# paulvantieghem/curla

Hardware: AMD Instinct MI355X
Metric: SAC+CURL gradient updates/sec, batch=512 84x84x9 (higher is better)
Workload: dtype f32

## Files before the change

curla_amd/_lib.py:

```python
import ctypes
import os

_HERE = os.path.dirname(os.path.abspath(__file__))
LIB_PATH = os.environ.get("CURLA_LIB_PATH") or os.path.join(_HERE, "libcurla_hip.so")

c_int, c_ll, c_float, c_size_t, vp = ctypes.c_int, ctypes.c_longlong, ctypes.c_float, ctypes.c_size_t, ctypes.c_void_p
c_u64 = ctypes.c_ulonglong
c_double = ctypes.c_double

ABI_VERSION = 8

SIGNATURES = {
    "curla_conv1_fwd": [vp, c_int, vp, vp, vp, vp, vp, vp, c_int, c_int, c_int, c_int, c_int, c_int, c_int, c_float, vp],
    "curla_conv3x3_s1_fwd": [vp, vp, vp, vp, c_int, c_int, c_int, c_int, vp],
    "curla_conv3x3_s1_fwd2": [vp, vp, vp, vp, c_int, vp, vp, vp, vp, c_int, c_int, c_int, c_int, vp],
    "curla_conv3x3_s1_fwd_stack": [c_int, vp, vp, vp, vp, c_int, vp, vp, vp, vp, c_int, c_int, c_int, c_int, vp],
    "curla_conv3x3_s1_stack_granule": [],
    "curla_conv1_fwd2": [vp, vp, vp, vp, vp, vp, vp, c_int, vp, vp, vp, vp, vp, vp, c_int, c_int, c_int, c_int, c_int, c_int,
                         c_int, c_float, vp],
    "curla_conv3x3_s1_dgrad": [vp, vp, vp, vp, c_int, c_int, c_int, c_int, vp],
    "curla_conv3x3_s1_wgrad": [vp, vp, vp, vp, vp, c_int, c_int, c_int, c_int, vp],
    "curla_conv1_wgrad": [vp, c_int, vp, vp, vp, vp, vp, vp, vp, c_int, c_int, c_int, c_int, c_int, c_int, c_int,
                          c_float, vp],
    "curla_conv3x3_s1_wgrad_slabs": [vp, vp, vp, c_int, c_int, c_int, c_int, vp, vp],
    "curla_conv1_wgrad_slabs": [vp, c_int, vp, vp, vp, vp, vp, c_int, c_int, c_int, c_int, c_int, c_int, c_int, c_float, vp,
                                vp],
    "curla_conv3x3_s1_bwd_slabs": [vp, vp, vp, vp, vp, c_int, c_int, c_int, c_int, vp, vp],
    "curla_conv1_dgrad": [vp, vp, vp, c_int, c_int, c_int, c_int, c_int, c_float, vp],
    "curla_wgrad_reduce_multi": [c_int, vp, vp, vp, vp, vp, vp, vp],
    "curla_conv_wgrad_workspace_floats": [c_int],
    "curla_gemm": [vp, c_int, c_int, c_ll, vp, c_int, c_int, c_ll, vp, c_int, c_ll, c_int, c_int, c_int, c_int, c_int,
                   c_ll, c_float, vp, c_ll, c_int, vp, c_int, c_ll, vp],
    "curla_fc_dx": [vp, vp, vp, vp, c_int, c_int, c_int, vp],
    "curla_fc_dw": [vp, vp, vp, c_int, c_int, c_int, vp],
    "curla_fc_bwd": [vp, vp, vp, vp, vp, c_int, c_int, c_int, vp],
    "curla_fc_bwd_ln": [vp, vp, vp, vp, vp, c_int, c_int, c_int, vp, c_int, vp, vp, vp, vp],
    "curla_fc_dw_ln": [vp, vp, vp, c_int, c_int, c_int, vp, c_int, vp, vp, vp, vp],
    "curla_fc_bwd_ln2": [vp, vp, vp, vp, vp, c_int, c_int, c_int, vp, c_int, vp, vp, vp, vp, c_int, c_int, vp, vp],
    "curla_curl_head": [vp, vp, vp, vp, vp, vp, c_int, c_int, vp, vp, vp, vp, vp, vp, vp, vp, vp, vp],
    "curla_gemm_nested": [vp, c_int, c_int, c_ll, c_ll, vp, c_int, c_int, c_ll, c_ll, vp, c_int, c_ll, c_ll, c_int, c_int, c_int,
                          c_int, c_int, c_float, vp, c_ll, c_ll, c_int, vp, c_int, c_ll, c_ll, vp],
    "curla_mlp_out_fwd_nested": [vp, c_ll, c_ll, vp, c_ll, c_ll, vp, c_ll, c_ll, vp, c_ll, c_ll, c_int, c_int, c_int, c_int, c_int,
                                 vp],
# ... 175 lines not shown
```

curla_amd/csrc/conv.hip:

```cpp
#include <algorithm>
#include <cstdlib>
#include <cstring>
#include <mutex>
#include <type_traits>

#include "common.h"
#include "options.h"

namespace {

constexpr int kLdsPix = 36;

enum { MODE_FWD = 0, MODE_DGRAD = 1 };

__device__ float g_zero_px[32];

#ifdef CURLA_ABLATE
int g_ablate = 0;
#define ABL(bit) (a.dbg & (bit))
#define ABL_HOST g_ablate
#else
#define ABL(bit) 0
#define ABL_HOST 0
#endif
// ... 23 lines not shown
    __syncthreads();
    rw43::run_layer<MODE_FWD, 4>(A.g[l], A.p[l][0], A.p[l][1], lds, blockIdx.x, gridDim.x);
    if (l + 1 < A.nlayers) {
      __builtin_amdgcn_fence(__ATOMIC_RELEASE, "workgroup");
      __syncthreads();
      __builtin_amdgcn_fence(__ATOMIC_ACQUIRE, "workgroup");
    }
  }
}

__global__ __launch_bounds__(256, 1) __attribute__((amdgpu_waves_per_eu(1, 1))) void conv_rw43_dgrad_kernel(rw::Args A) {
  extern __shared__ __attribute__((aligned(16))) float lds[];
  rw43::build_filter<MODE_DGRAD, 256>(lds, A.p[0][0].w, nullptr, threadIdx.x);
  __syncthreads();
  rw43::run_layer<MODE_DGRAD, 4>(A.g[0], A.p[0][0], A.p[0][1], lds, blockIdx.x, gridDim.x);
}

#include "conv_rwb.h"

#ifdef RWB_CLOCK
__device__ unsigned long long g_rwb_clock[3 * 1024];
#endif

template <int NW>
__device__ __forceinline__ void rwb_fwd_body(const rw::Args& A) {
  extern __shared__ __attribute__((aligned(16))) unsigned short lds_h[];
#if defined(RWB_STAMP) || defined(RWB_CLOCK)
  const unsigned long long kt0 = __builtin_readcyclecounter(), kr0 = __builtin_amdgcn_s_memrealtime();
#endif
  for (int l = 0; l < A.nlayers; ++l) {
#ifdef RWB_STAMP
    const unsigned long long k0 = __builtin_readcyclecounter();
#endif
    rwb::build_filter<MODE_FWD, 64 * NW>(lds_h, A.p[l][0].w, A.p[l][1].B > 0 ? A.p[l][1].w : nullptr, threadIdx.x);
    __syncthreads();
#ifdef RWB_STAMP
    const unsigned long long k1 = __builtin_readcyclecounter();
#endif
    rwb::run_layer<MODE_FWD, NW>(A.g[l], A.p[l][0], A.p[l][1], lds_h, blockIdx.x, gridDim.x);
#ifdef RWB_STAMP
    const unsigned long long k2 = __builtin_readcyclecounter();
#endif
    if (l + 1 < A.nlayers) {
      __builtin_amdgcn_fence(__ATOMIC_RELEASE, "workgroup");
      __syncthreads();
      __builtin_amdgcn_fence(__ATOMIC_ACQUIRE, "workgroup");
    }
#ifdef RWB_STAMP
    const unsigned long long k3 = __builtin_readcyclecounter();
    if (threadIdx.x == 0 && blockIdx.x == 7) {
      rwb::g_rwb_stamp[4] += k1 - k0, rwb::g_rwb_stamp[5] += k2 - k1, rwb::g_rwb_stamp[6] += k3 - k2, rwb::g_rwb_stamp[7] += 1;
    }
#endif
  }
#ifdef RWB_STAMP
  if (threadIdx.x == 0 && blockIdx.x == 7) {
    rwb::g_rwb_stamp[15] += __builtin_readcyclecounter() - kt0;
    rwb::g_rwb_stamp[14] += __builtin_amdgcn_s_memrealtime() - kr0;
  }
#endif
#ifdef RWB_CLOCK
  if (threadIdx.x == 0 && blockIdx.x < 1024) {
    g_rwb_clock[3 * blockIdx.x + 0] += __builtin_readcyclecounter() - kt0;
    g_rwb_clock[3 * blockIdx.x + 1] += __builtin_amdgcn_s_memrealtime() - kr0;
    g_rwb_clock[3 * blockIdx.x + 2] += 1;
  }
#endif
}

__global__ __launch_bounds__(512, 1) void conv_rwb_fwd_kernel(rw::Args A) { rwb_fwd_body<8>(A); }

__global__ __launch_bounds__(512, 1) void conv_rwb_dgrad_kernel(rw::Args A) {
  extern __shared__ __attribute__((aligned(16))) unsigned short lds_h[];
  rwb::build_filter<MODE_DGRAD, 512>(lds_h, A.p[0][0].w, nullptr, threadIdx.x);
  __syncthreads();
  rwb::run_layer<MODE_DGRAD, 8>(A.g[0], A.p[0][0], A.p[0][1], lds_h, blockIdx.x, gridDim.x);
}

__global__ __launch_bounds__(256, 2) void conv_rw_dgrad_kernel(rw::Args A) {
  extern __shared__ __attribute__((aligned(16))) float lds[];
  rw::build_filter<MODE_DGRAD, 256>(lds, A.p[0][0].w, nullptr, threadIdx.x);
  __syncthreads();
  rw::run_layer<MODE_DGRAD, 4>(A.g[0], A.p[0][0], A.p[0][1], lds, blockIdx.x, gridDim.x);
}

#include "conv1_rw.h"

template <int C>
__global__ __launch_bounds__(512, 2) void conv1_rw_fwd_kernel(rw::Conv1Args a) {
  rw::conv1_body<C, 8>(a, blockIdx.x, gridDim.x);
}

template <int C>
__global__ __launch_bounds__(512, 2) void wgrad1_rw_kernel(rw::Wgrad1Args a) {
  rw::wgrad1_body<C, 8>(a, blockIdx.x, gridDim.x);
}

// ... 44 lines not shown
    rw::wgrad_body<4>(wa, bid, nblk);
}

__global__ __launch_bounds__(256, 2) void wgrad_rw_kernel(rw::WgradArgs wa) {
  wgrad_any(wa, blockIdx.x, gridDim.x);
}

__global__ __launch_bounds__(256, 2) void bwd_rw2_kernel(rw::WgradArgs wa, rw::Args da, int nw) {
  if ((int)blockIdx.x < nw) {
    wgrad_any(wa, blockIdx.x, nw);
  } else {
    extern __shared__ __attribute__((aligned(16))) float lds[];
    rw::build_filter<MODE_DGRAD, 256>(lds, da.p[0][0].w, nullptr, threadIdx.x);
    __syncthreads();
    rw::run_layer<MODE_DGRAD, 4>(da.g[0], da.p[0][0], da.p[0][1], lds, (int)blockIdx.x - nw, (int)gridDim.x - nw);
  }
}

__global__ __launch_bounds__(256, 2) void bwd_rwb2_kernel(rw::WgradArgs wa, rw::Args da, int nw) {
  if ((int)blockIdx.x < nw) {
    wgrad_any(wa, blockIdx.x, nw);
  } else {
    extern __shared__ __attribute__((aligned(16))) unsigned short lds_hb[];
    rwb::build_filter<MODE_DGRAD, 256>(lds_hb, da.p[0][0].w, nullptr, threadIdx.x);
    __syncthreads();
    rwb::run_layer<MODE_DGRAD, 4>(da.g[0], da.p[0][0], da.p[0][1], lds_hb, (int)blockIdx.x - nw, (int)gridDim.x - nw);
  }
}

#include "conv1_wgrad.h"

#include "conv_wgrad_reduce.h"

constexpr int kMaxLds = 160 * 1024;
static_assert(2 * rwb::kWBytes <= kMaxLds, "the two problems' split filters of conv_rwb_fwd_kernel must fit one CU's LDS");
template <typename K>
int set_lds(K kernel, size_t bytes) {
  if (bytes > (size_t)kMaxLds) return CURLA_ERR_UNSUPPORTED;
  return curla_set_dyn_lds(reinterpret_cast<const void*>(kernel), kMaxLds);
}

template <typename... Params, typename... Args>
int launch(void (*kernel)(Params...), int grid, int threads, size_t lds, hipStream_t st, const Args&... args) {
  if (lds) {
    const int rc = set_lds(kernel, lds);
    if (rc != CURLA_OK) return rc;
  }
// ... 53 lines not shown
  return one_band && Wc * C <= 64 * 16 && opt != kConv1U8Band ? Conv1U8Form::Hybrid : Conv1U8Form::Band;
}

enum class Conv1F32Form { Rw, Band };
Conv1F32Form select_conv1_f32_form(int src_kind, int C, int Hc, int Wc) {
  const bool rw = src_kind == kSrcF32Nhwc && curla_opt(kOptConv1F32) == kConv1F32Rw && (long long)Hc * Wc * C * 4 < (1LL << 30);
  return rw ? Conv1F32Form::Rw : Conv1F32Form::Band;
}

enum class Wgrad1U8Form { B16, F32, F32FourWave };
constexpr size_t kWgrad1U8BandBudget = 76 * 1024, kWgrad1U8BandBudget4 = 38 * 1024;
Wgrad1U8Form select_wgrad1_u8_form(int C, int Wc, int Wo) {
  if ((ABL_HOST & 1024) && (size_t)(2 * 4 + 1) * u8_row_bytes(Wc, C) <= kWgrad1U8BandBudget4) return Wgrad1U8Form::F32FourWave;
  return curla_opt(kOptWgrad1U8) != kWgrad1U8F32 && Wo >= 8 && 3 * C <= 32 ? Wgrad1U8Form::B16 : Wgrad1U8Form::F32;
}

bool rw_supported(int Hi, int Wi) { return (long long)(Hi + 2) * (Wi + 2) * 128 < (1LL << 30); }

rw::Geom s1_plan(S1Form f, int Hi, int Wi, int Ho, int Wo) {
  return f == S1Form::B3 ? rwb::plan(Hi, Wi, Ho, Wo) : f == S1Form::F43 ? rw43::plan(Hi, Wi, Ho, Wo) : rw::plan(Hi, Wi, Ho, Wo);
}
size_t s1_filter_bytes(S1Form f) {
  return f == S1Form::B3 ? rwb::kWBytes : (f == S1Form::F43 ? rw43::kWFloats : rw::kWFloats) * sizeof(float);
}

int launch_rw_fwd(int nlayers, const float* in, const float* const* w, const float* const* bias, float* const* out, int B,
                  const float* in2, const float* const* w2, const float* const* bias2, float* const* out2, int B2, int Hi,
                  int Wi, bool owned, hipStream_t st) {
  const S1Form form = select_s1_form();
  rw::Args A;
  A.nlayers = nlayers;
  for (int l = 0; l < rw::kMaxLayers; ++l) {
    const bool on = l < nlayers;
    const int hi = Hi - 2 * l, wi = Wi - 2 * l;
    A.g[l] = on ? s1_plan(form, hi, wi, hi - 2, wi - 2) : rw::Geom{};
    A.p[l][0] = on ? rw::Problem{l == 0 ? in : out[l - 1], w[l], bias[l], out[l], B} : rw::Problem{};
    A.p[l][1] = (on && B2 > 0) ? rw::Problem{l == 0 ? in2 : out2[l - 1], w2[l], bias2[l], out2[l], B2} : rw::Problem{};
    if (on && (hi < 3 || wi < 3)) return CURLA_ERR_UNSUPPORTED;
  }
  if (!rw_supported(Hi, Wi)) return CURLA_ERR_UNSUPPORTED;
  const int cus = curla_cu_count();
  const int grid = owned ? cus : std::min(B > B2 ? B : B2, cus);
  const size_t lds = (size_t)(B2 > 0 ? 2 : 1) * s1_filter_bytes(form);
  switch (form) {
    case S1Form::B3: return launch(conv_rwb_fwd_kernel, grid, 512, lds, st, A);
    case S1Form::F43: return launch(conv_rw43_fwd_kernel, grid, 256, lds, st, A);
    default: return launch(conv_rw_fwd_kernel, grid, 512, lds, st, A);
  }
}

rw::Args rw_dgrad_args(S1Form form, const float* g, const float* w, const float* act_below, float* gin, int B, int Ho,
                       int Wo) {
  rw::Args A;
  A.nlayers = 1;
  for (int l = 0; l < rw::kMaxLayers; ++l) A.g[l] = rw::Geom{}, A.p[l][0] = rw::Problem{}, A.p[l][1] = rw::Problem{};
  A.g[0] = s1_plan(form, Ho, Wo, Ho + 2, Wo + 2);
  A.p[0][0] = rw::Problem{g, w, act_below, gin, B};
  return A;
}

int launch_dgrad(S1Form form, const float* g, const float* w, const float* act_below, float* gin, int B, int Ho, int Wo,
                 hipStream_t st) {
  const rw::Args A = rw_dgrad_args(form, g, w, act_below, gin, B, Ho, Wo);
  const int cus = curla_cu_count();
  const size_t lds = s1_filter_bytes(form);
  switch (form) {
    case S1Form::B3: return launch(conv_rwb_dgrad_kernel, std::min(B, cus), 512, lds, st, A);
    case S1Form::F43: return launch(conv_rw43_dgrad_kernel, std::min(B, cus), 256, lds, st, A);
    default: return launch(conv_rw_dgrad_kernel, std::min(B, 2 * cus), 256, lds, st, A);
  }
}

int launch_conv_s1(int mode, const float* in, const float* w, const float* aux, float* out, int B, int Hs, int Ws,
                   hipStream_t st, const float* in2 = nullptr, const float* w2 = nullptr, const float* aux2 = nullptr,
                   float* out2 = nullptr, int B2 = 0) {
  if (!rw_supported(Hs, Ws)) return CURLA_ERR_UNSUPPORTED;
  if (mode == MODE_FWD) return launch_rw_fwd(1, in, &w, &aux, &out, B, in2, &w2, &aux2, &out2, B2, Hs, Ws, false, st);
  return launch_dgrad(select_s1_form(), in, w, aux, out, B, Hs, Ws, st);
}

rw::WgradArgs wgrad_args(const float* in, const float* g, float* workspace, int B, int Hi, int Wi, int Ho, int Wo) {
  const bool two_d = select_s1_wgrad_form() == S1WgradForm::XY;
  return rw::WgradArgs{in, g, workspace, B, Hi, Wi, Ho, Wo, two_d ? rw::plan4p(Hi, Wi, Ho, Wo) : rw::plan4(Hi, Wi, Ho, Wo),
                       two_d ? 1 : 0};
}

// ... 149 lines not shown
  return launch_conv_s1(MODE_FWD, in, w, bias, out, B, Hi, Wi, static_cast<hipStream_t>(stream), in2, w2, bias2, out2, B2);
}

int curla_conv3x3_s1_fwd_stack(int nlayers, const float* in, const float* const* w, const float* const* bias,
                               float* const* out, int B, const float* in2, const float* const* w2,
                               const float* const* bias2, float* const* out2, int B2, int Hi, int Wi, int channels,
                               void* stream) {
  CURLA_REQUIRE(nlayers > 0 && nlayers <= rw::kMaxLayers && in && w && bias && out && B > 0 && Hi >= 3 && Wi >= 3);
  CURLA_REQUIRE(B2 == 0 || (in2 && w2 && bias2 && out2));
  if (channels != 32) return CURLA_ERR_UNSUPPORTED;
  const int G1 = curla_cu_count();
  if (B % G1 != 0 || B2 % G1 != 0) return CURLA_ERR_UNSUPPORTED;
  CURLA_REQUIRE(aligned16(in) && (!B2 || aligned16(in2)));
  for (int l = 0; l < nlayers; ++l) {
    CURLA_REQUIRE(w[l] && bias[l] && out[l] && aligned16(w[l]) && aligned16(bias[l]) && aligned16(out[l]));
    CURLA_REQUIRE(!B2 || (w2[l] && bias2[l] && out2[l] && aligned16(w2[l]) && aligned16(bias2[l]) && aligned16(out2[l])));
  }
  if (Hi - 2 * nlayers < 1 || Wi - 2 * nlayers < 1) return CURLA_ERR_UNSUPPORTED;
  return launch_rw_fwd(nlayers, in, w, bias, out, B, in2, w2, bias2, out2, B2, Hi, Wi, true,
                       static_cast<hipStream_t>(stream));
}

int curla_conv3x3_s1_stack_granule(void) { return curla_cu_count(); }

int curla_conv3x3_s1_dgrad(const float* g, const float* w, const float* act_below, float* gin, int B, int Ho, int Wo,
                           int channels, void* stream) {
  CURLA_REQUIRE(g && w && act_below && gin && B > 0 && Ho >= 1 && Wo >= 1);
  if (channels != 32) return gen_dgrad(g, w, act_below, gin, B, Ho, Wo, channels, static_cast<hipStream_t>(stream));
  CURLA_REQUIRE(aligned16(g) && aligned16(gin) && aligned16(act_below) && aligned16(w));
  return launch_conv_s1(MODE_DGRAD, g, w, act_below, gin, B, Ho, Wo, static_cast<hipStream_t>(stream));
}

static int conv1_common_check(const void* src, int src_kind, int B, int C, int Hs, int Ws, int Hc, int Wc) {
  CURLA_REQUIRE(src && B > 0 && Hc >= 3 && Wc >= 3 && src_kind >= 0 && src_kind <= 2);
  if (C != 9 && C != 12 && C != 6 && C != 3) return CURLA_ERR_UNSUPPORTED;
  if (src_kind == kSrcU8Ring) {
    CURLA_REQUIRE(Hs >= Hc && Ws >= Wc);
    CURLA_REQUIRE((reinterpret_cast<uintptr_t>(src) & 3) == 0);
  }
  return CURLA_OK;
}

struct Conv1Second {
  const int64_t* idx;
  const int32_t* h1;
  const int32_t* w1;
// ... 144 lines not shown
  CURLA_REQUIRE(nslabs);
  return launch_wgrad_s1(in, g, workspace, B, Hi, Wi, channels, static_cast<hipStream_t>(stream), nslabs);
}

int curla_conv3x3_s1_bwd_slabs(const float* in, const float* g, const float* w, float* gin, float* workspace, int B, int Hi,
                               int Wi, int channels, int* nslabs, void* stream) {
  CURLA_REQUIRE(in && g && w && gin && workspace && nslabs && B > 0 && Hi >= 3 && Wi >= 3);
  hipStream_t st = static_cast<hipStream_t>(stream);
  if (channels != 32) {
    const int rc = gen_wgrad_s1(in, g, workspace, B, Hi, Wi, channels, st, nslabs);
    return rc != CURLA_OK ? rc : gen_dgrad(g, w, in, gin, B, Hi - 2, Wi - 2, channels, st);
  }
  CURLA_REQUIRE(aligned16(in) && aligned16(g) && aligned16(w) && aligned16(gin));
  const int Ho = Hi - 2, Wo = Wi - 2;
  if (!rw_supported(Hi, Wi)) return CURLA_ERR_UNSUPPORTED;
  const S1Form form = select_s1_form();
  if (form == S1Form::F43) {
    const int rc = launch_wgrad_s1(in, g, workspace, B, Hi, Wi, channels, st, nslabs);
    return rc != CURLA_OK ? rc : launch_dgrad(form, g, w, in, gin, B, Ho, Wo, st);
  }
  const int per_cu = select_bwd_shape(form, B, Ho, Wo) == BwdShape::SideBySide ? 1 : 2;
  const int n = std::min(B, per_cu * curla_cu_count());
  const rw::WgradArgs wr = wgrad_args(in, g, workspace, B, Hi, Wi, Ho, Wo);
  const rw::Args dr = rw_dgrad_args(form, g, w, in, gin, B, Ho, Wo);
  const size_t lds = std::max<size_t>(s1_filter_bytes(form), kPartialS1 * sizeof(float));
  *nslabs = n;
  return launch(form == S1Form::B3 ? bwd_rwb2_kernel : bwd_rw2_kernel, 2 * n, 256, lds, st, wr, dr, n);
}

int curla_wgrad_reduce_multi(int njobs, const float* const* slabs, const int* nslabs, const int* nw, const int* nb,
                             float* const* dw, float* const* db, void* stream) {
  CURLA_REQUIRE(njobs > 0 && njobs <= kMaxReduceJobs && slabs && nslabs && nw && dw && db);
  ReduceJobs J;
  int blocks = 0;
  for (int j = 0; j < njobs; ++j) {
    CURLA_REQUIRE(slabs[j] && dw[j] && db[j] && nslabs[j] > 0 && nw[j] > 0);
    J.partial[j] = slabs[j], J.dw[j] = dw[j], J.db[j] = db[j], J.nslabs[j] = nslabs[j], J.nw[j] = nw[j];
    J.nb[j] = nb ? nb[j] : 32;
    CURLA_REQUIRE(J.nb[j] > 0);
    J.first_block[j] = blocks;
    blocks += (nw[j] + J.nb[j] + 31) / 32;
  }
  J.first_block[njobs] = blocks;
  J.njobs = njobs;
  return launch(wgrad_reduce_multi_kernel, blocks, 1024, 0, static_cast<hipStream_t>(stream), J);
}

// ... 71 lines not shown
```

curla_amd/csrc/conv_rw.h:

```cpp
#pragma once

namespace rw {

constexpr int kWFloats = 3 * 4 * 2 * 2 * 256;

__device__ __forceinline__ __amdgpu_buffer_rsrc_t uniform_rsrc(const void* p, int bytes) {
  const unsigned long long a = reinterpret_cast<unsigned long long>(p);
  const unsigned lo32 = __builtin_amdgcn_readfirstlane((unsigned)a);
  const unsigned hi32 = __builtin_amdgcn_readfirstlane((unsigned)(a >> 32));
  return __builtin_amdgcn_make_buffer_rsrc(reinterpret_cast<void*>(((unsigned long long)hi32 << 32) | lo32), (short)0,
                                           __builtin_amdgcn_readfirstlane(bytes), 0x00020000);
}

struct Geom {
  int Hi, Wi;
  int Ho, Wo;
  int nfull;
  int brem;
  int nr;
  int nseg;
  int ntr;
  int steps;
};

struct Problem {
  const float* in;
  const float* w;
  const float* aux;
  float* out;
  int B;
};

constexpr int kMaxLayers = 6;
struct Args {
  int nlayers;
  Geom g[kMaxLayers];
  Problem p[kMaxLayers][2];
};

inline void plan_units(Geom& g, int Ho, int cols, int per) {
  g.nfull = cols / per, g.brem = cols % per;
  g.nr = g.nseg = g.ntr = 0;
  if (g.brem) {
    long best = -1;
    for (int nr = 1; nr <= Ho; ++nr) {
      const int nseg = (Ho + nr - 1) / nr;
      const int ntr = (g.brem * nseg + per - 1) / per;
      const long cost = (long)ntr * nr * 64 + (long)ntr * 2 * 8;
      if (best < 0 || cost <= best) best = cost, g.nr = nr, g.nseg = nseg, g.ntr = ntr;
    }
  }
  g.steps = g.nfull * Ho + g.ntr * g.nr;
}

inline Geom plan(int Hi, int Wi, int Ho, int Wo) {
  Geom g;
  g.Hi = Hi, g.Wi = Wi, g.Ho = Ho, g.Wo = Wo;
  plan_units(g, Ho, (Wo + 1) / 2, 16);
  return g;
}
// ... 228 lines not shown
```

curla_amd/csrc/conv_rwb.h:

```cpp
#pragma once

namespace rwb {

using rw::Args;
using rw::Geom;
using rw::Problem;
using rw::uniform_rsrc;

typedef short bf16x8 __attribute__((ext_vector_type(8)));
typedef unsigned u32x4 __attribute__((ext_vector_type(4)));
typedef __bf16 bf16x2_t __attribute__((ext_vector_type(2)));

constexpr int kWBytes = 3 * 4 * 2 * 3 * 64 * 16;

inline Geom plan(int Hi, int Wi, int Ho, int Wo) { return rw::plan(Hi, Wi, Ho, Wo); }

struct B3 {
  u32x4 h, m, l;
};

__device__ __forceinline__ unsigned cvt_pk_bf16(float x0, float x1) {
  const f32x2 v = {x0, x1};
  return __builtin_bit_cast(unsigned, __builtin_convertvector(v, bf16x2_t));
}
// ... 2 lines not shown
  B3 o;
#if defined(RWB_ABL) && (RWB_ABL & 1)
#pragma unroll
  for (int p = 0; p < 4; ++p) o.h[p] = __builtin_bit_cast(unsigned, v[2 * p]), o.m[p] = __builtin_bit_cast(unsigned, v[2 * p + 1]);
  o.l = o.h;
  return o;
#endif
#pragma unroll
  for (int p = 0; p < 4; ++p) {
    const float x0 = v[2 * p], x1 = v[2 * p + 1];
    const unsigned h = cvt_pk_bf16(x0, x1);
    const float r0 = x0 - __builtin_bit_cast(float, h << 16), r1 = x1 - __builtin_bit_cast(float, h & 0xFFFF0000u);
    const unsigned m = cvt_pk_bf16(r0, r1);
    const float s0 = r0 - __builtin_bit_cast(float, m << 16), s1 = r1 - __builtin_bit_cast(float, m & 0xFFFF0000u);
    o.h[p] = h, o.m[p] = m, o.l[p] = cvt_pk_bf16(s0, s1);
  }
  return o;
}

__device__ __forceinline__ f32x4 mfma_bf16(const u32x4 a, const u32x4 b, const f32x4 c) {
  return __builtin_amdgcn_mfma_f32_16x16x32_bf16(__builtin_bit_cast(bf16x8, a), __builtin_bit_cast(bf16x8, b), c, 0, 0, 0);
}

template <int MODE, int NT>
__device__ __forceinline__ void build_filter(unsigned short* lds_w, const float* __restrict__ w0,
                                             const float* __restrict__ w1, int tid) {
  const int nitems = (w1 ? 2 : 1) * 6 * 64;
  for (int item = tid; item < nitems; item += NT) {
    const int slot = item & 63, dm = (item >> 6) % 6, prob = item / 384;
    const int li = slot & 15, kq = slot >> 4, dy = dm >> 1, mt = dm & 1;
    const float* __restrict__ w = prob ? w1 : w0;
    const int co = 16 * mt + li;
    float u[8][4];
#pragma unroll
    for (int j = 0; j < 8; ++j) {
      const int ci = 8 * kq + j;
      const float* t = MODE == MODE_FWD ? w + (co * 32 + ci) * 9 + dy * 3 : w + (ci * 32 + co) * 9 + (2 - dy) * 3;
      if (MODE == MODE_FWD)
        rw::filter_transform(t[0], t[1], t[2], u[j]);
      else
        rw::filter_transform(t[2], t[1], t[0], u[j]);
    }
    u32x4* img = reinterpret_cast<u32x4*>(lds_w + prob * (kWBytes / 2));
#pragma unroll
    for (int pos = 0; pos < 4; ++pos) {
      float v[8];
#pragma unroll
      for (int j = 0; j < 8; ++j) v[j] = u[j][pos];
      const B3 x = split8(v);
      u32x4* p = img + ((((dy * 4 + pos) * 2 + mt) * 3)) * 64 + slot;
      p[0] = x.h, p[64] = x.m, p[128] = x.l;
    }
  }
}

#ifdef RWB_STAMP
__device__ unsigned long long g_rwb_stamp[16];
#endif

struct Acc {
  f32x4 m[2][4];
};

template <int MODE, int NW>
__device__ __forceinline__ void run_layer(const Geom& G, const Problem& P0, const Problem& P1, const unsigned short* lds_w,
                                          int bid, int nblk) {
  const int lane = threadIdx.x & 63;
  const int wave = __builtin_amdgcn_readfirstlane(threadIdx.x >> 6);
  const int li = lane & 15, kq = lane >> 4;
  const int pad = MODE == MODE_FWD ? 0 : 2;
  const int cnt0 = bid < P0.B ? (P0.B - bid + nblk - 1) / nblk : 0;
  const int cnt1 = bid < P1.B ? (P1.B - bid + nblk - 1) / nblk : 0;
  const int nstrips = G.nfull + G.ntr;
  const int T = (cnt0 + cnt1) * G.steps;
  const int lo = (int)((long)wave * T / NW), hi = (int)((long)(wave + 1) * T / NW);
  const int in_row = G.Wi * 128, out_row = G.Wo * 128;

// ... 192 lines not shown
```

curla_amd/csrc/options.h:

```cpp
#pragma once

enum CurlaOpt {
  kOptConv1U8 = 0,
  kOptConv1F32,
  kOptS1Fwd,
  kOptBwdSplit,
  kOptGemmTile,
  kOptLinearBwd,
  kOptGemmMfma,
  kOptS1Wgrad,
  kOptWgrad1U8,
  kOptCount
};

enum Conv1U8Opt { kConv1U8Auto, kConv1U8Hybrid, kConv1U8Band, kConv1U8Rw, kConv1U8Rwb, kConv1U8Values };
enum Conv1F32Opt { kConv1F32Rw, kConv1F32Band, kConv1F32Values };
enum S1FwdOpt { kS1FwdAuto, kS1FwdF23, kS1FwdF43, kS1FwdB3, kS1FwdValues };
enum BwdSplitOpt { kBwdSplitAuto, kBwdSplitOff, kBwdSplitOn, kBwdSplitValues };
enum GemmTileOpt { kGemmTileAuto, kGemmTile6464, kGemmTile6432, kGemmTile3232, kGemmTile12864, kGemmTileValues };
enum LinearBwdOpt { kLinearBwdPair, kLinearBwdSplit, kLinearBwdValues };
enum GemmMfmaOpt { kGemmMfmaAuto, kGemmMfmaF32, kGemmMfmaB3, kGemmMfmaValues };
enum S1WgradOpt { kS1WgradAuto, kS1WgradX, kS1WgradXY, kS1WgradValues };
enum Wgrad1U8Opt { kWgrad1U8Auto, kWgrad1U8F32, kWgrad1U8B16, kWgrad1U8Values };

int curla_opt(int id);
```

curla_amd/csrc/options.hip:

```cpp
#include "options.h"

#include <atomic>
#include <cctype>
#include <cstdlib>
#include <cstring>
#include <mutex>

#include "../../include/curla_hip.h"

namespace {

struct OptDef {
  const char* name;
  const char* values[6];
  const char* alias[6];
};

constexpr OptDef kDefs[kOptCount] = {
    {"conv1_u8", {"auto", "hybrid", "band", "rw", "rwb", nullptr}, {nullptr, nullptr, nullptr, nullptr, nullptr, nullptr}},
    {"conv1_f32", {"rw", "band", nullptr}, {nullptr, nullptr, nullptr}},
    {"s1_fwd", {"auto", "f23", "f43", "b3", nullptr}, {nullptr, nullptr, nullptr, "bf16x3", nullptr}},
    {"bwd_split", {"auto", "0", "1", nullptr}, {nullptr, "off", "on", nullptr}},
    {"gemm_tile", {"auto", "6464", "6432", "3232", "12864", nullptr}, {nullptr, "64x64", "64x32", "32x32", "128x64", nullptr}},
    {"linear_bwd", {"pair", "split", nullptr}, {nullptr, nullptr, nullptr}},
    {"gemm_mfma", {"auto", "f32", "b3", nullptr}, {nullptr, nullptr, "bf16x3", nullptr}},
    {"s1_wgrad", {"auto", "x", "xy", nullptr}, {nullptr, "1d", "2d", nullptr}},
    {"wgrad1_u8", {"auto", "f32", "b16", nullptr}, {nullptr, nullptr, "bf16", nullptr}},
};

constexpr int kValueCount[kOptCount] = {kConv1U8Values, kConv1F32Values, kS1FwdValues, kBwdSplitValues, kGemmTileValues,
                                        kLinearBwdValues, kGemmMfmaValues, kS1WgradValues, kWgrad1U8Values};
constexpr bool value_counts_match() {
  for (int id = 0; id < kOptCount; ++id)
    if (!kDefs[id].values[kValueCount[id] - 1] || kDefs[id].values[kValueCount[id]]) return false;
  return true;
}
static_assert(value_counts_match(), "options.h names a different number of values than kDefs lists for some option");

std::atomic<int> g_value[kOptCount];
std::once_flag g_once;

int parse(const OptDef& d, const char* text) {
  for (int i = 0; i < 6 && d.values[i]; ++i)
    if (!strcmp(text, d.values[i]) || (d.alias[i] && !strcmp(text, d.alias[i]))) return i;
  return -1;
}

void init_from_env() {
  for (int id = 0; id < kOptCount; ++id) {
    char env[64] = "CURLA_";
    size_t n = strlen(env);
    for (const char* p = kDefs[id].name; *p && n + 1 < sizeof(env); ++p) env[n++] = (char)toupper((unsigned char)*p);
    env[n] = 0;
    const char* e = getenv(env);
// ... 39 lines not shown
```

curla_amd/curl_sac.py:

```python
import os
import warnings

import numpy as np
import torch
import torch.nn as nn

from . import autograd, ops
from .augmentations import RandomCrop
from .encoder import CNNEncoder
from .ops import ObsRef
from .optim import FlatAdam

LOG_FREQ = 25_000


def weight_init(m):
    if isinstance(m, nn.Linear):
        nn.init.orthogonal_(m.weight.data)
        if m.bias is not None:
            m.bias.data.zero_()
        return
    if isinstance(m, (nn.Conv2d, nn.ConvTranspose2d)):
        kh, kw = m.weight.shape[2:]
        assert kh == kw, "square kernels only"
# ... 699 lines not shown
        B, F, K, L = obs_ref.B, enc.feature_dim, enc.flat_dim, enc.num_layers
        acts = ws.acts_main
        dy, dy2 = (dz, None) if twin_ld is None else (dz[0], dz[1])
        streams = ops.fc_bwd_streams(F, K)
        ln = ln_token if ln_token is not None else ops.ln_bwd(
            dy, xhat, rstd, enc.ln.weight, B, F, ws.dfc, dgamma=enc.ln.weight.grad, dbeta=enc.ln.bias.grad,
            dbias_in=enc.fc.bias.grad, dy2=dy2, ld=twin_ld, defer=ws.ln_partial if streams else None)
        h = acts[-1]
        cur = L % 2
        g = ws.gviews[cur][L - 1]
        if streams and conv_grads:
            ops.fc_bwd(ws.dfc, enc.fc.weight, h, g, enc.fc.weight.grad, B, F, K, ln=ln)
        elif streams:
            ops.fc_dw(ws.dfc, h, enc.fc.weight.grad, B, F, K, ln=ln)
        else:
            ops.linear_dw(ws.dfc, 0, h, 0, enc.fc.weight.grad, 0, B, F, K)
        if dense_done is not None:
            dense_done()
        if not conv_grads:
            return
        if not streams:
            ops.linear_dx(ws.dfc, 0, enc.fc.weight, 0, g, 0, B, F, K, mask=h)
        jobs = []
        for layer in range(L, 1, -1):
            conv = enc.convs[layer - 1]
            cur ^= 1
            gin = ws.gviews[cur][layer - 2]
            n = ops.conv_s1_bwd_slabs(acts[layer - 2], g, conv.weight, gin, ws.wg_ws[layer - 1])
            jobs.append((ws.wg_ws[layer - 1], n, conv.weight.grad, conv.bias.grad))
            g = gin
        n = ops.conv1_wgrad_slabs(obs_ref, g, ws.wg_ws[0], enc.num_filters)
        jobs.append((ws.wg_ws[0], n, enc.convs[0].weight.grad, enc.convs[0].bias.grad))
        for i in range(0, len(jobs), 8):
            ops.wgrad_reduce_multi(jobs[i:i + 8])

    def _records(self, step):
        return self.log_param_hist_imgs and step % LOG_FREQ == 0

    def _noise(self, ws, noise):
        if noise is not None:
            ws.noise.copy_(noise)
            return ws.noise, None
        if self._graph_cap is not None:
            cap = self._graph_cap
            addr = cap["rng"][cap["n_noise"]]
            cap["n_noise"] += 1
# ... 564 lines not shown
```

curla_amd/ops.py:

```python
import ctypes

import torch

from . import _lib
from ._lib import call, ptr, stream

F32 = torch.float32


def _dev(t, dtype=F32):
    if not ((t.is_cuda or _lib._trace_hook is not None) and t.dtype == dtype and t.is_contiguous()):
        raise _lib.CurlaHipError(f"expected a contiguous {dtype} CUDA tensor, got {t.dtype} {t.device} "
                                 f"contiguous={t.is_contiguous()}")
    return t


class ObsRef:

    __slots__ = ("src", "is_u8", "idx", "h1", "w1", "B", "C", "Hs", "Ws", "Hc", "Wc", "guard", "pair")

    def __init__(self):
        self.guard = None
        self.pair = None

# ... 99 lines not shown
def cu_count():
    if _lib._trace_hook is not None:
        return 256
    return _device_cached("cus", lambda: torch.cuda.get_device_properties(torch.cuda.current_device()).multi_processor_count)


def conv1_pairable(o1: "ObsRef", o2: "ObsRef"):
    return (o1.is_u8 == 1 and o2.is_u8 == 1 and o1.src.data_ptr() == o2.src.data_ptr() and o1.src.shape == o2.src.shape
            and (o1.Hc, o1.Wc) == (o2.Hc, o2.Wc))


def conv1_fwd2(o1: "ObsRef", w, b, out, o2: "ObsRef", w2, b2, out2, scale=1.0 / 255.0):
    o1.check(), o2.check()
    call("curla_conv1_fwd2", ptr(o1.src), ptr(o1.idx), ptr(o1.h1), ptr(o1.w1), ptr(w), ptr(b), ptr(out), o1.B, ptr(o2.idx),
         ptr(o2.h1), ptr(o2.w1), ptr(w2), ptr(b2), ptr(out2), o2.B, o1.C, o1.Hs, o1.Ws, o1.Hc, o1.Wc, w.shape[0], scale,
         stream())


def conv_s1_dgrad(g, w, act_below, gin):
    B, H, W, C = g.shape
    call("curla_conv3x3_s1_dgrad", ptr(g), ptr(w), ptr(act_below), ptr(gin), B, H, W, C, stream())


def conv_s1_wgrad(x, g, dw, db, ws):
    B, H, W, C = x.shape
    call("curla_conv3x3_s1_wgrad", ptr(x), ptr(g), ptr(dw), ptr(db), ptr(ws), B, H, W, C, stream())


def conv_s1_wgrad_slabs(x, g, ws):
    import ctypes
    B, H, W, C = x.shape
    n = ctypes.c_int(1)
    call("curla_conv3x3_s1_wgrad_slabs", ptr(x), ptr(g), ptr(ws), B, H, W, C, ctypes.addressof(n), stream())
    return n.value


def conv_s1_bwd_slabs(x, g, w, gin, ws):
    import ctypes
    B, H, W, C = x.shape
    n = ctypes.c_int(1)
    call("curla_conv3x3_s1_bwd_slabs", ptr(x), ptr(g), ptr(w), ptr(gin), ptr(ws), B, H, W, C, ctypes.addressof(n),
         stream())
    return n.value


def conv1_wgrad_slabs(obs: ObsRef, g, ws, channels, scale=1.0 / 255.0):
# ... 486 lines not shown
```

include/curla_hip.h:

```cpp
#ifndef CURLA_HIP_H
#define CURLA_HIP_H

#include <stddef.h>
#include <stdint.h>

#ifdef __cplusplus
extern "C" {
#endif

#define CURLA_OK 0
#define CURLA_ERR_ARG (-1)
#define CURLA_ERR_LAUNCH (-2)
#define CURLA_ERR_UNSUPPORTED (-3)

const char* curla_version(void);

#define CURLA_ABI_VERSION 8
int curla_abi_version(void);

int curla_set_option(const char* name, const char* value);
const char* curla_get_option(const char* name);


int curla_conv1_fwd(const void* src, int src_kind, const int64_t* idx, const int32_t* h1, const int32_t* w1,
// ... 9 lines not shown
int curla_conv3x3_s1_fwd2(const float* in, const float* w, const float* bias, float* out, int B, const float* in2,
                          const float* w2, const float* bias2, float* out2, int B2, int Hi, int Wi, int channels,
                          void* stream);
int curla_conv3x3_s1_fwd_stack(int nlayers, const float* in, const float* const* w, const float* const* bias,
                               float* const* out, int B, const float* in2, const float* const* w2,
                               const float* const* bias2, float* const* out2, int B2, int Hi, int Wi, int channels,
                               void* stream);
int curla_conv3x3_s1_stack_granule(void);

int curla_conv3x3_s1_dgrad(const float* g, const float* w, const float* act_below, float* gin, int B, int Ho, int Wo,
                           int channels, void* stream);
int curla_conv3x3_s1_wgrad(const float* in, const float* g, float* dw, float* db, float* workspace, int B, int Hi,
                           int Wi, int channels, void* stream);
int curla_conv1_wgrad(const void* src, int src_kind, const int64_t* idx, const int32_t* h1, const int32_t* w1,
                      const float* g, float* dw, float* db, float* workspace, int B, int C, int Hs, int Ws, int Hc,
                      int Wc, int channels, float scale, void* stream);
int curla_conv3x3_s1_wgrad_slabs(const float* in, const float* g, float* workspace, int B, int Hi, int Wi, int channels,
                                 int* nslabs, void* stream);
int curla_conv1_wgrad_slabs(const void* src, int src_kind, const int64_t* idx, const int32_t* h1, const int32_t* w1,
                            const float* g, float* workspace, int B, int C, int Hs, int Ws, int Hc, int Wc, int channels,
                            float scale, int* nslabs, void* stream);
int curla_conv3x3_s1_bwd_slabs(const float* in, const float* g, const float* w, float* gin, float* workspace, int B, int Hi,
                               int Wi, int channels, int* nslabs, void* stream);
int curla_conv1_dgrad(const float* g, const float* w, float* dobs, int B, int C, int H, int W, int channels,
                      float scale, void* stream);
int curla_wgrad_reduce_multi(int njobs, const float* const* slabs, const int* nslabs, const int* nw, const int* nb,
                             float* const* dw, float* const* db, void* stream);
size_t curla_conv_wgrad_workspace_floats(int cin);

int curla_gemm(const float* A, int a_kmajor, int lda, long long strideA, const float* B, int b_kmajor, int ldb,
               long long strideB, float* C, int ldc, long long strideC, int M, int N, int K, int nbatch, int ksplit,
               long long split_stride, float alpha, const float* bias, long long strideBias, int relu,
               const float* mask, int ldmask, long long strideMask, void* stream);
int curla_gemm_small_shape(int M, int N, int K, int nbatch);
int curla_gemm_colsum(const float* A, int a_kmajor, int lda, long long strideA, const float* B, int b_kmajor, int ldb,
                      long long strideB, float* C, int ldc, long long strideC, int M, int N, int K, int nbatch,
                      float* colsum, long long strideColsum, void* stream);
int curla_linear_bwd(const float* dy, long long stride_dy, const float* x, long long stride_x, const float* W,
                     long long stride_W, const float* mask, long long stride_mask, float* dW, long long stride_dW,
                     float* db, long long stride_db, float* dx, long long stride_dx, int B, int N, int K, int nbatch,
                     void* stream);
int curla_gemm_nested(const float* A, int a_kmajor, int lda, long long strideA, long long strideA2, const float* B,
                      int b_kmajor, int ldb, long long strideB, long long strideB2, float* C, int ldc, long long strideC,
                      long long strideC2, int M, int N, int K, int nbatch, int nbatch2, float alpha, const float* bias,
                      long long strideBias, long long strideBias2, int relu, const float* mask, int ldmask,
                      long long strideMask, long long strideMask2, void* stream);
// ... 176 lines not shown
```

Before: 516.7.

## Presplit bf16x3 conv filter images in a separate kernel and copy into LDS

Moves the per-workgroup filter transform and bf16x3 split for the 3x3 stride-1 convolutions into a small standalone kernel that writes split filter images to a per-stream workspace. The fused conv kernels now copy those images into LDS instead of rebuilding them in every block. In the forward stack the next layer's image is fetched before the layer barrier, so the global loads overlap the sync. Dgrad filters for all backward layers are prepared in one launch ahead of the backward loop. This adds extra kernel launches, a host-side workspace registry with mutex and capture-key bookkeeping, and extra global memory traffic.

After: 520.2, median of 3. No clear change (+0.7%).

```diff
diff --git a/curla_amd/_lib.py b/curla_amd/_lib.py
--- a/curla_amd/_lib.py
+++ b/curla_amd/_lib.py
@@ -19,6 +19,7 @@
     "curla_conv1_fwd2": [vp, vp, vp, vp, vp, vp, vp, c_int, vp, vp, vp, vp, vp, vp, c_int, c_int, c_int, c_int, c_int, c_int,
                          c_int, c_float, vp],
     "curla_conv3x3_s1_dgrad": [vp, vp, vp, vp, c_int, c_int, c_int, c_int, vp],
+    "curla_conv3x3_s1_dgrad_prepare": [c_int, vp, c_int, vp],
     "curla_conv3x3_s1_wgrad": [vp, vp, vp, vp, vp, c_int, c_int, c_int, c_int, vp],
     "curla_conv1_wgrad": [vp, c_int, vp, vp, vp, vp, vp, vp, vp, c_int, c_int, c_int, c_int, c_int, c_int, c_int,
                           c_float, vp],
diff --git a/curla_amd/csrc/conv.hip b/curla_amd/csrc/conv.hip
--- a/curla_amd/csrc/conv.hip
+++ b/curla_amd/csrc/conv.hip
@@ -69,35 +69,74 @@
 __device__ unsigned long long g_rwb_clock[3 * 1024];
 #endif
 
+__device__ __forceinline__ void layer_barrier() {
+  __builtin_amdgcn_fence(__ATOMIC_RELEASE, "workgroup");
+  __syncthreads();
+  __builtin_amdgcn_fence(__ATOMIC_ACQUIRE, "workgroup");
+}
+
+template <int NT, int NIMG, bool BARRIER>
+__device__ __forceinline__ void rwb_copy_filter(unsigned short* lds_w, const unsigned short* img) {
+  int tid = threadIdx.x;
+  asm volatile("" : "+v"(tid));
+  rwb::FilterCopy<NT, NIMG> cp;
+  cp.fetch(img, tid);
+  if (BARRIER) layer_barrier();
+  cp.store(lds_w, tid);
+}
+
 template <int NW>
 __device__ __forceinline__ void rwb_fwd_body(const rw::Args& A) {
   extern __shared__ __attribute__((aligned(16))) unsigned short lds_h[];
 #if defined(RWB_STAMP) || defined(RWB_CLOCK)
   const unsigned long long kt0 = __builtin_readcyclecounter(), kr0 = __builtin_amdgcn_s_memrealtime();
 #endif
+  const int nprob = A.p[0][1].B > 0 ? 2 : 1;
+#ifdef RWB_STAMP
+  unsigned long long k0 = __builtin_readcyclecounter();
+#endif
+  if (A.img) {
+    if (nprob > 1)
+      rwb_copy_filter<64 * NW, 2, false>(lds_h, A.img);
+    else
+      rwb_copy_filter<64 * NW, 1, false>(lds_h, A.img);
+  } else {
+    rwb::build_filter<MODE_FWD, 64 * NW>(lds_h, A.p[0][0].w, nprob > 1 ? A.p[0][1].w : nullptr, threadIdx.x);
+  }
+  __syncthreads();
   for (int l = 0; l < A.nlayers; ++l) {
-#ifdef RWB_STAMP
-    const unsigned long long k0 = __builtin_readcyclecounter();
-#endif
-    rwb::build_filter<MODE_FWD, 64 * NW>(lds_h, A.p[l][0].w, A.p[l][1].B > 0 ? A.p[l][1].w : nullptr, threadIdx.x);
-    __syncthreads();
 #ifdef RWB_STAMP
     const unsigned long long k1 = __builtin_readcyclecounter();
 #endif
     rwb::run_layer<MODE_FWD, NW>(A.g[l], A.p[l][0], A.p[l][1], lds_h, blockIdx.x, gridDim.x);
 #ifdef RWB_STAMP
     const unsigned long long k2 = __builtin_readcyclecounter();
+    unsigned long long k3 = k2;
 #endif
     if (l + 1 < A.nlayers) {
-      __builtin_amdgcn_fence(__ATOMIC_RELEASE, "workgroup");
+      if (A.img) {
+        const unsigned short* next = A.img + (size_t)(l + 1) * nprob * (rwb::kWBytes / 2);
+        if (nprob > 1)
+          rwb_copy_filter<64 * NW, 2, true>(lds_h, next);
+        else
+          rwb_copy_filter<64 * NW, 1, true>(lds_h, next);
+#ifdef RWB_STAMP
+        k3 = __builtin_readcyclecounter();
+#endif
+      } else {
+        layer_barrier();
+#ifdef RWB_STAMP
+        k3 = __builtin_readcyclecounter();
+#endif
+        rwb::build_filter<MODE_FWD, 64 * NW>(lds_h, A.p[l + 1][0].w, nprob > 1 ? A.p[l + 1][1].w : nullptr, threadIdx.x);
+      }
       __syncthreads();
-      __builtin_amdgcn_fence(__ATOMIC_ACQUIRE, "workgroup");
     }
 #ifdef RWB_STAMP
-    const unsigned long long k3 = __builtin_readcyclecounter();
     if (threadIdx.x == 0 && blockIdx.x == 7) {
       rwb::g_rwb_stamp[4] += k1 - k0, rwb::g_rwb_stamp[5] += k2 - k1, rwb::g_rwb_stamp[6] += k3 - k2, rwb::g_rwb_stamp[7] += 1;
     }
+    k0 = k3;
 #endif
   }
 #ifdef RWB_STAMP
@@ -117,9 +156,29 @@
 
 __global__ __launch_bounds__(512, 1) void conv_rwb_fwd_kernel(rw::Args A) { rwb_fwd_body<8>(A); }
 
+constexpr int kMaxImages = 2 * rw::kMaxLayers;
+struct FilterJobs {
+  const float* w[kMaxImages];
+};
+template <int MODE>
+__global__ __launch_bounds__(64) void split_filter_kernel(FilterJobs J, unsigned short* img) {
+  const int k = blockIdx.x / 6, dm = blockIdx.x % 6;
+  rwb::build_filter_item<MODE>(reinterpret_cast<rwb::u32x4*>(img + (size_t)k * (rwb::kWBytes / 2)), J.w[k],
+                               dm * 64 + (int)threadIdx.x);
+}
+
+template <int NT>
+__device__ __forceinline__ void rwb_dgrad_filter(unsigned short* lds_w, const rw::Args& A) {
+  if (A.img) {
+    rwb_copy_filter<NT, 1, false>(lds_w, A.img);
+  } else {
+    rwb::build_filter<MODE_DGRAD, NT>(lds_w, A.p[0][0].w, nullptr, threadIdx.x);
+  }
+}
+
 __global__ __launch_bounds__(512, 1) void conv_rwb_dgrad_kernel(rw::Args A) {
   extern __shared__ __attribute__((aligned(16))) unsigned short lds_h[];
-  rwb::build_filter<MODE_DGRAD, 512>(lds_h, A.p[0][0].w, nullptr, threadIdx.x);
+  rwb_dgrad_filter<512>(lds_h, A);
   __syncthreads();
   rwb::run_layer<MODE_DGRAD, 8>(A.g[0], A.p[0][0], A.p[0][1], lds_h, blockIdx.x, gridDim.x);
 }
@@ -210,7 +269,7 @@
     wgrad_any(wa, blockIdx.x, nw);
   } else {
     extern __shared__ __attribute__((aligned(16))) unsigned short lds_hb[];
-    rwb::build_filter<MODE_DGRAD, 256>(lds_hb, da.p[0][0].w, nullptr, threadIdx.x);
+    rwb_dgrad_filter<256>(lds_hb, da);
     __syncthreads();
     rwb::run_layer<MODE_DGRAD, 4>(da.g[0], da.p[0][0], da.p[0][1], lds_hb, (int)blockIdx.x - nw, (int)gridDim.x - nw);
   }
@@ -310,6 +369,109 @@
 }
 size_t s1_filter_bytes(S1Form f) {
   return f == S1Form::B3 ? rwb::kWBytes : (f == S1Form::F43 ? rw43::kWFloats : rw::kWFloats) * sizeof(float);
+}
+
+enum class S1Filters { Presplit, Build };
+S1Filters select_s1_filters() { return curla_opt(kOptS1Filters) == kS1FiltersBuild ? S1Filters::Build : S1Filters::Presplit; }
+
+constexpr int kMaxPrepared = rw::kMaxLayers;
+constexpr int kFwdSlot = 0, kPreparedSlot = kMaxImages, kLoneSlot = kPreparedSlot + kMaxPrepared;
+constexpr size_t kWorkspaceBytes = (size_t)(kLoneSlot + 1) * rwb::kWBytes;
+constexpr int kMaxWorkspaces = 64;
+
+struct PreparedImage {
+  const float* w;
+  int slot;
+  unsigned long long capture;
+};
+struct S1Workspace {
+  int dev;
+  hipStream_t st;
+  unsigned short* buf;
+  int nprepared;
+  PreparedImage prepared[kMaxPrepared];
+};
+std::mutex g_s1_ws_mu;
+S1Workspace g_s1_ws[kMaxWorkspaces];
+int g_s1_nws = 0;
+
+unsigned long long capture_key(hipStream_t st) {
+  hipStreamCaptureStatus cs = hipStreamCaptureStatusNone;
+  unsigned long long id = 0;
+  if (hipStreamGetCaptureInfo(st, &cs, &id) != hipSuccess) {
+    (void)hipGetLastError();
+    return ~0ULL;
+  }
+  return cs == hipStreamCaptureStatusNone ? 0 : cs == hipStreamCaptureStatusActive ? id + 1 : ~0ULL;
+}
+
+S1Workspace* s1_workspace(hipStream_t st) {
+  int dev = 0;
+  if (hipGetDevice(&dev) != hipSuccess) return nullptr;
+  for (int i = 0; i < g_s1_nws; ++i)
+    if (g_s1_ws[i].dev == dev && g_s1_ws[i].st == st) return &g_s1_ws[i];
+  if (g_s1_nws == kMaxWorkspaces || capture_key(st) != 0) return nullptr;
+  void* p = nullptr;
+  if (hipMalloc(&p, kWorkspaceBytes) != hipSuccess) {
+    (void)hipGetLastError();
+    return nullptr;
+  }
+  g_s1_ws[g_s1_nws] = S1Workspace{dev, st, static_cast<unsigned short*>(p), 0, {}};
+  return &g_s1_ws[g_s1_nws++];
+}
+
+int launch_split_filters(int mode, const FilterJobs& J, int n, unsigned short* img, hipStream_t st) {
+  return mode == MODE_FWD ? launch(split_filter_kernel<MODE_FWD>, 6 * n, 64, 0, st, J, img)
+                          : launch(split_filter_kernel<MODE_DGRAD>, 6 * n, 64, 0, st, J, img);
+}
+
+int s1_fwd_images(const FilterJobs& J, int n, hipStream_t st, const unsigned short** img) {
+  *img = nullptr;
+  if (select_s1_filters() == S1Filters::Build) return CURLA_OK;
+  std::lock_guard<std::mutex> lock(g_s1_ws_mu);
+  S1Workspace* ws = s1_workspace(st);
+  if (!ws) return CURLA_OK;
+  ws->nprepared = 0;
+  *img = ws->buf + (size_t)kFwdSlot * (rwb::kWBytes / 2);
+  return launch_split_filters(MODE_FWD, J, n, ws->buf + (size_t)kFwdSlot * (rwb::kWBytes / 2), st);
+}
+
+int s1_dgrad_prepare(int n, const float* const* w, hipStream_t st) {
+  if (select_s1_filters() == S1Filters::Build) return CURLA_OK;
+  std::lock_guard<std::mutex> lock(g_s1_ws_mu);
+  S1Workspace* ws = s1_workspace(st);
+  if (!ws) return CURLA_OK;
+  ws->nprepared = 0;
+  const unsigned long long key = capture_key(st);
+  if (key == ~0ULL) return CURLA_OK;
+  FilterJobs J{};
+  for (int i = 0; i < n; ++i) J.w[i] = w[i];
+  const int rc = launch_split_filters(MODE_DGRAD, J, n, ws->buf + (size_t)kPreparedSlot * (rwb::kWBytes / 2), st);
+  if (rc != CURLA_OK) return rc;
+  for (int i = 0; i < n; ++i) ws->prepared[i] = PreparedImage{w[i], kPreparedSlot + i, key};
+  ws->nprepared = n;
+  return CURLA_OK;
+}
+
+int s1_dgrad_image(const float* w, hipStream_t st, const unsigned short** img) {
+  *img = nullptr;
+  if (select_s1_filters() == S1Filters::Build) return CURLA_OK;
+  std::lock_guard<std::mutex> lock(g_s1_ws_mu);
+  S1Workspace* ws = s1_workspace(st);
+  if (!ws) return CURLA_OK;
+  if (ws->nprepared) {
+    const unsigned long long key = capture_key(st);
+    for (int i = 0; i < ws->nprepared; ++i)
+      if (ws->prepared[i].w == w && ws->prepared[i].capture == key) {
+        *img = ws->buf + (size_t)ws->prepared[i].slot * (rwb::kWBytes / 2);
+        ws->prepared[i] = ws->prepared[--ws->nprepared];
+        return CURLA_OK;
+      }
+  }
+  FilterJobs J{};
+  J.w[0] = w;
+  *img = ws->buf + (size_t)kLoneSlot * (rwb::kWBytes / 2);
+  return launch_split_filters(MODE_DGRAD, J, 1, ws->buf + (size_t)kLoneSlot * (rwb::kWBytes / 2), st);
 }
 
 int launch_rw_fwd(int nlayers, const float* in, const float* const* w, const float* const* bias, float* const* out, int B,
@@ -330,6 +492,16 @@
   const int cus = curla_cu_count();
   const int grid = owned ? cus : std::min(B > B2 ? B : B2, cus);
   const size_t lds = (size_t)(B2 > 0 ? 2 : 1) * s1_filter_bytes(form);
+  if (form == S1Form::B3) {
+    FilterJobs J{};
+    int n = 0;
+    for (int l = 0; l < nlayers; ++l) {
+      J.w[n++] = w[l];
+      if (B2 > 0) J.w[n++] = w2[l];
+    }
+    const int rc = s1_fwd_images(J, n, st, &A.img);
+    if (rc != CURLA_OK) return rc;
+  }
   switch (form) {
     case S1Form::B3: return launch(conv_rwb_fwd_kernel, grid, 512, lds, st, A);
     case S1Form::F43: return launch(conv_rw43_fwd_kernel, grid, 256, lds, st, A);
@@ -349,7 +521,11 @@
 
 int launch_dgrad(S1Form form, const float* g, const float* w, const float* act_below, float* gin, int B, int Ho, int Wo,
                  hipStream_t st) {
-  const rw::Args A = rw_dgrad_args(form, g, w, act_below, gin, B, Ho, Wo);
+  rw::Args A = rw_dgrad_args(form, g, w, act_below, gin, B, Ho, Wo);
+  if (form == S1Form::B3) {
+    const int rc = s1_dgrad_image(w, st, &A.img);
+    if (rc != CURLA_OK) return rc;
+  }
   const int cus = curla_cu_count();
   const size_t lds = s1_filter_bytes(form);
   switch (form) {
@@ -545,6 +721,13 @@
 }
 
 int curla_conv3x3_s1_stack_granule(void) { return curla_cu_count(); }
+
+int curla_conv3x3_s1_dgrad_prepare(int nlayers, const float* const* w, int channels, void* stream) {
+  CURLA_REQUIRE(nlayers > 0 && nlayers <= kMaxPrepared && w);
+  for (int l = 0; l < nlayers; ++l) CURLA_REQUIRE(w[l] && aligned16(w[l]));
+  if (channels != 32 || select_s1_form() != S1Form::B3) return CURLA_OK;
+  return s1_dgrad_prepare(nlayers, w, static_cast<hipStream_t>(stream));
+}
 
 int curla_conv3x3_s1_dgrad(const float* g, const float* w, const float* act_below, float* gin, int B, int Ho, int Wo,
                            int channels, void* stream) {
@@ -735,7 +918,11 @@
   const int per_cu = select_bwd_shape(form, B, Ho, Wo) == BwdShape::SideBySide ? 1 : 2;
   const int n = std::min(B, per_cu * curla_cu_count());
   const rw::WgradArgs wr = wgrad_args(in, g, workspace, B, Hi, Wi, Ho, Wo);
-  const rw::Args dr = rw_dgrad_args(form, g, w, in, gin, B, Ho, Wo);
+  rw::Args dr = rw_dgrad_args(form, g, w, in, gin, B, Ho, Wo);
+  if (form == S1Form::B3) {
+    const int rc = s1_dgrad_image(w, st, &dr.img);
+    if (rc != CURLA_OK) return rc;
+  }
   const size_t lds = std::max<size_t>(s1_filter_bytes(form), kPartialS1 * sizeof(float));
   *nslabs = n;
   return launch(form == S1Form::B3 ? bwd_rwb2_kernel : bwd_rw2_kernel, 2 * n, 256, lds, st, wr, dr, n);
diff --git a/curla_amd/csrc/conv_rw.h b/curla_amd/csrc/conv_rw.h
--- a/curla_amd/csrc/conv_rw.h
+++ b/curla_amd/csrc/conv_rw.h
@@ -36,6 +36,7 @@
   int nlayers;
   Geom g[kMaxLayers];
   Problem p[kMaxLayers][2];
+  const unsigned short* img = nullptr;
 };
 
 inline void plan_units(Geom& g, int Ho, int cols, int per) {
diff --git a/curla_amd/csrc/conv_rwb.h b/curla_amd/csrc/conv_rwb.h
--- a/curla_amd/csrc/conv_rwb.h
+++ b/curla_amd/csrc/conv_rwb.h
@@ -48,37 +48,59 @@
   return __builtin_amdgcn_mfma_f32_16x16x32_bf16(__builtin_bit_cast(bf16x8, a), __builtin_bit_cast(bf16x8, b), c, 0, 0, 0);
 }
 
+constexpr int kWItems = 6 * 64;
+template <int MODE>
+__device__ __forceinline__ void build_filter_item(u32x4* img, const float* __restrict__ w, int item) {
+  const int slot = item & 63, dm = item >> 6;
+  const int li = slot & 15, kq = slot >> 4, dy = dm >> 1, mt = dm & 1;
+  const int co = 16 * mt + li;
+  float u[8][4];
+#pragma unroll
+  for (int j = 0; j < 8; ++j) {
+    const int ci = 8 * kq + j;
+    const float* t = MODE == MODE_FWD ? w + (co * 32 + ci) * 9 + dy * 3 : w + (ci * 32 + co) * 9 + (2 - dy) * 3;
+    if (MODE == MODE_FWD)
+      rw::filter_transform(t[0], t[1], t[2], u[j]);
+    else
+      rw::filter_transform(t[2], t[1], t[0], u[j]);
+  }
+#pragma unroll
+  for (int pos = 0; pos < 4; ++pos) {
+    float v[8];
+#pragma unroll
+    for (int j = 0; j < 8; ++j) v[j] = u[j][pos];
+    const B3 x = split8(v);
+    u32x4* p = img + ((((dy * 4 + pos) * 2 + mt) * 3)) * 64 + slot;
+    p[0] = x.h, p[64] = x.m, p[128] = x.l;
+  }
+}
+
 template <int MODE, int NT>
 __device__ __forceinline__ void build_filter(unsigned short* lds_w, const float* __restrict__ w0,
                                              const float* __restrict__ w1, int tid) {
-  const int nitems = (w1 ? 2 : 1) * 6 * 64;
+  const int nitems = (w1 ? 2 : 1) * kWItems;
   for (int item = tid; item < nitems; item += NT) {
-    const int slot = item & 63, dm = (item >> 6) % 6, prob = item / 384;
-    const int li = slot & 15, kq = slot >> 4, dy = dm >> 1, mt = dm & 1;
-    const float* __restrict__ w = prob ? w1 : w0;
-    const int co = 16 * mt + li;
-    float u[8][4];
-#pragma unroll
-    for (int j = 0; j < 8; ++j) {
-      const int ci = 8 * kq + j;
-      const float* t = MODE == MODE_FWD ? w + (co * 32 + ci) * 9 + dy * 3 : w + (ci * 32 + co) * 9 + (2 - dy) * 3;
-      if (MODE == MODE_FWD)
-        rw::filter_transform(t[0], t[1], t[2], u[j]);
-      else
-        rw::filter_transform(t[2], t[1], t[0], u[j]);
-    }
-    u32x4* img = reinterpret_cast<u32x4*>(lds_w + prob * (kWBytes / 2));
-#pragma unroll
-    for (int pos = 0; pos < 4; ++pos) {
-      float v[8];
-#pragma unroll
-      for (int j = 0; j < 8; ++j) v[j] = u[j][pos];
-      const B3 x = split8(v);
-      u32x4* p = img + ((((dy * 4 + pos) * 2 + mt) * 3)) * 64 + slot;
-      p[0] = x.h, p[64] = x.m, p[128] = x.l;
-    }
-  }
-}
+    const int prob = item / kWItems;
+    build_filter_item<MODE>(reinterpret_cast<u32x4*>(lds_w + prob * (kWBytes / 2)), prob ? w1 : w0, item - prob * kWItems);
+  }
+}
+
+template <int NT, int NIMG>
+struct FilterCopy {
+  static constexpr int kVec = NIMG * (kWBytes / 16), kPer = kVec / NT;
+  static_assert(kVec % NT == 0, "a workgroup copies an image in whole rounds of its threads");
+  u32x4 r[kPer];
+  __device__ __forceinline__ void fetch(const unsigned short* img, int tid) {
+    const u32x4* src = reinterpret_cast<const u32x4*>(img) + tid;
+#pragma unroll
+    for (int i = 0; i < kPer; ++i) r[i] = src[i * NT];
+  }
+  __device__ __forceinline__ void store(unsigned short* lds_w, int tid) const {
+    u32x4* dst = reinterpret_cast<u32x4*>(lds_w) + tid;
+#pragma unroll
+    for (int i = 0; i < kPer; ++i) dst[i * NT] = r[i];
+  }
+};
 
 #ifdef RWB_STAMP
 __device__ unsigned long long g_rwb_stamp[16];
diff --git a/curla_amd/csrc/options.h b/curla_amd/csrc/options.h
--- a/curla_amd/csrc/options.h
+++ b/curla_amd/csrc/options.h
@@ -10,6 +10,7 @@
   kOptGemmMfma,
   kOptS1Wgrad,
   kOptWgrad1U8,
+  kOptS1Filters,
   kOptCount
 };
 
@@ -22,5 +23,6 @@
 enum GemmMfmaOpt { kGemmMfmaAuto, kGemmMfmaF32, kGemmMfmaB3, kGemmMfmaValues };
 enum S1WgradOpt { kS1WgradAuto, kS1WgradX, kS1WgradXY, kS1WgradValues };
 enum Wgrad1U8Opt { kWgrad1U8Auto, kWgrad1U8F32, kWgrad1U8B16, kWgrad1U8Values };
+enum S1FiltersOpt { kS1FiltersAuto, kS1FiltersPresplit, kS1FiltersBuild, kS1FiltersValues };
 
 int curla_opt(int id);
diff --git a/curla_amd/csrc/options.hip b/curla_amd/csrc/options.hip
--- a/curla_amd/csrc/options.hip
+++ b/curla_amd/csrc/options.hip
@@ -26,10 +26,12 @@
     {"gemm_mfma", {"auto", "f32", "b3", nullptr}, {nullptr, nullptr, "bf16x3", nullptr}},
     {"s1_wgrad", {"auto", "x", "xy", nullptr}, {nullptr, "1d", "2d", nullptr}},
     {"wgrad1_u8", {"auto", "f32", "b16", nullptr}, {nullptr, nullptr, "bf16", nullptr}},
+    {"s1_filters", {"auto", "presplit", "build", nullptr}, {nullptr, nullptr, nullptr, nullptr}},
 };
 
 constexpr int kValueCount[kOptCount] = {kConv1U8Values, kConv1F32Values, kS1FwdValues, kBwdSplitValues, kGemmTileValues,
-                                        kLinearBwdValues, kGemmMfmaValues, kS1WgradValues, kWgrad1U8Values};
+                                        kLinearBwdValues, kGemmMfmaValues, kS1WgradValues, kWgrad1U8Values,
+                                        kS1FiltersValues};
 constexpr bool value_counts_match() {
   for (int id = 0; id < kOptCount; ++id)
     if (!kDefs[id].values[kValueCount[id] - 1] || kDefs[id].values[kValueCount[id]]) return false;
diff --git a/curla_amd/curl_sac.py b/curla_amd/curl_sac.py
--- a/curla_amd/curl_sac.py
+++ b/curla_amd/curl_sac.py
@@ -745,6 +745,7 @@
         if not streams:
             ops.linear_dx(ws.dfc, 0, enc.fc.weight, 0, g, 0, B, F, K, mask=h)
         jobs = []
+        ops.conv_s1_dgrad_prepare([enc.convs[layer - 1].weight for layer in range(L, 1, -1)])
         for layer in range(L, 1, -1):
             conv = enc.convs[layer - 1]
             cur ^= 1
diff --git a/curla_amd/ops.py b/curla_amd/ops.py
--- a/curla_amd/ops.py
+++ b/curla_amd/ops.py
@@ -145,6 +145,14 @@
     call("curla_conv3x3_s1_dgrad", ptr(g), ptr(w), ptr(act_below), ptr(gin), B, H, W, C, stream())
 
 
+def conv_s1_dgrad_prepare(weights):
+    n = len(weights)
+    if n == 0 or n > 6:
+        return
+    arr = (ctypes.c_void_p * n)(*[ptr(w) for w in weights])
+    call("curla_conv3x3_s1_dgrad_prepare", n, ctypes.addressof(arr), weights[0].shape[0], stream())
+
+
 def conv_s1_wgrad(x, g, dw, db, ws):
     B, H, W, C = x.shape
     call("curla_conv3x3_s1_wgrad", ptr(x), ptr(g), ptr(dw), ptr(db), ptr(ws), B, H, W, C, stream())
diff --git a/include/curla_hip.h b/include/curla_hip.h
--- a/include/curla_hip.h
+++ b/include/curla_hip.h
@@ -55,6 +55,7 @@
                             float scale, int* nslabs, void* stream);
 int curla_conv3x3_s1_bwd_slabs(const float* in, const float* g, const float* w, float* gin, float* workspace, int B, int Hi,
                                int Wi, int channels, int* nslabs, void* stream);
+int curla_conv3x3_s1_dgrad_prepare(int nlayers, const float* const* w, int channels, void* stream);
 int curla_conv1_dgrad(const float* g, const float* w, float* dobs, int B, int C, int H, int W, int channels,
                       float scale, void* stream);
 int curla_wgrad_reduce_multi(int njobs, const float* const* slabs, const int* nslabs, const int* nw, const int* nb,
```
